# naver/multi-hmr

Measured on AMD Instinct MI355X. Metric: images/sec (whole node) ViT-L 896x896 bs32, higher is better.
Workload: dtype f16; 1 GPU; multiHMR_896_L full forward: dinov2_vitl14 896x896, 32 images/GPU, 8 pinned persons/image -> HPH (depth 2) -> SMPL-X LBS; image-sharded x1; global_batch=32, parallelism=dp1 (images)

## Files before the change

multi_hmr_amd/csrc/attention.hip:

```cpp
#include <stdlib.h>
#include <type_traits>
#include "mhmr_common.h"
#include "mhmr_internal.h"

namespace {

__device__ __forceinline__ float max_lane32(float v) {
    const auto r = __builtin_amdgcn_permlane32_swap(__float_as_uint(v), __float_as_uint(v), false, false);
    return fmaxf(__uint_as_float(r[0]), __uint_as_float(r[1]));
}

constexpr int KB = 64;
#ifndef MHMR_ATTN_DEFAULT_VARIANT
#define MHMR_ATTN_DEFAULT_VARIANT 6
#endif
constexpr int KV_TILE_BYTES = KB * 64 * 2;
constexpr float BAND = 8.f;

template <int DT, int NW, int RING, int MODE>
__device__ __forceinline__ void attn_body(
    const void* __restrict__ qk_, const void* __restrict__ vt_, void* __restrict__ out_, int T, int Tp, int C, int H, int nqt,
    float limit, int* __restrict__ flags, int ldo, int o8, const int bid) {
    typedef typename Op<DT>::T Tt;
    typedef typename Op<DT>::V8 V8;
    typedef typename Op<DT>::V4 V4;
    extern __shared__ __attribute__((aligned(16))) char smem[];

    const int tid = threadIdx.x, lane = tid & 63;
    const int w = __builtin_amdgcn_readfirstlane(tid >> 6);
    const int hi = lane >> 5, l31 = lane & 31;

    const int qt = bid % nqt, bh = bid / nqt;
    const int b = bh / H, h = bh - b * H;
    constexpr int QB = 32 * NW;
    if (qt * QB >= T) {
        if constexpr (MODE == 3) {
            if (lane == 0) flags[4 * bid + w] = 0;
        }
        return;
    }

    const Tt* qk = (const Tt*)qk_;
    const Tt* vt = (const Tt*)vt_;
    const int ldq = 2 * C;
    const size_t row0 = (size_t)b * Tp;

    const int q_row = qt * QB + 32 * w + l31;
    const bool active = qt * QB + 32 * w < T;
    const bool in_buf = qt * QB + 32 * w < Tp;
    V8 qf[4] = {};
    if (in_buf) {
        const Tt* qp = qk + (row0 + q_row) * ldq + h * 64 + 8 * hi;
#pragma unroll
        for (int ks = 0; ks < 4; ++ks) qf[ks] = *(const V8*)(qp + 16 * ks);
        if (q_row >= T) {
#pragma unroll
            for (int ks = 0; ks < 4; ++ks) qf[ks] = V8{};
        }
    }

    constexpr int PASSES = 8 / NW, ROWS_PER_PASS = 8 * NW;
    constexpr int OPS = 2 * PASSES;
    const int srow = tid >> 3;
    const int schunk = (tid & 7) ^ ((tid >> 4) & 7);
    const Tt* k_src = qk + (row0 + srow) * ldq + C + h * 64 + schunk * 8;
    const Tt* v_src = vt + ((size_t)(b * H + h) * 64 + srow) * Tp + schunk * 8;
    auto stage = [&](int j, int buf) {
        char* sk = smem + buf * (2 * KV_TILE_BYTES) + w * 1024;
        char* sv = sk + KV_TILE_BYTES;
        const Tt* kp = k_src + (size_t)j * KB * ldq;
        const Tt* vp = v_src + j * KB;
#pragma unroll
        for (int ps = 0; ps < PASSES; ++ps) glds16(kp + (size_t)(ROWS_PER_PASS * ps) * ldq, sk + ps * (ROWS_PER_PASS * 128));
#pragma unroll
        for (int ps = 0; ps < PASSES; ++ps) glds16(vp + (size_t)(ROWS_PER_PASS * ps) * Tp, sv + ps * (ROWS_PER_PASS * 128));
    };

    const int fsw = (lane >> 1) & 7;

    f32x16 o[2];
#pragma unroll
    for (int i = 0; i < 2; ++i)
#pragma unroll
        for (int r = 0; r < 16; ++r) o[i][r] = 0.f;
    float m_ref = MODE == 1 ? -1e30f : 0.f, r_run = -INFINITY, l_run = 0.f;
    bool bad = false;

    const bool tail1 = MODE == 3 && (T & (KB - 1)) == 1 && T > KB;
    const int ntile = tail1 ? T / KB : (T + KB - 1) / KB;
#pragma unroll
    for (int t = 0; t < RING - 1; ++t) stage(t < ntile ? t : ntile - 1, t);
    int buf = 0, nbuf = RING - 1;
    for (int j = 0; j < ntile; ++j) {
        if constexpr (RING == 2) asm volatile("s_waitcnt vmcnt(0) lgkmcnt(0)" ::: "memory");
        else if constexpr (OPS * (RING - 2) == 2) asm volatile("s_waitcnt vmcnt(2) lgkmcnt(0)" ::: "memory");
        else if constexpr (OPS * (RING - 2) == 4) asm volatile("s_waitcnt vmcnt(4) lgkmcnt(0)" ::: "memory");
        else if constexpr (OPS * (RING - 2) == 6) asm volatile("s_waitcnt vmcnt(6) lgkmcnt(0)" ::: "memory");
        else asm volatile("s_waitcnt vmcnt(8) lgkmcnt(0)" ::: "memory");
        static_assert(OPS * (RING - 2) <= 8, "extend the counted waits");
        __builtin_amdgcn_s_barrier();
        __builtin_amdgcn_sched_barrier(0);
        const char* sk = smem + buf * (2 * KV_TILE_BYTES);
        const char* sv = sk + KV_TILE_BYTES;
        const int nbuf_now = nbuf;
        buf = buf == RING - 1 ? 0 : buf + 1;
        nbuf = nbuf == RING - 1 ? 0 : nbuf + 1;
        if (!active) {
            stage(j + RING - 1 < ntile ? j + RING - 1 : ntile - 1, nbuf_now);
            continue;
        }
        f32x16 s[2];
        {
            const float init = MODE == 1 ? 0.f : -m_ref;
#pragma unroll
            for (int sub = 0; sub < 2; ++sub)
#pragma unroll
                for (int r = 0; r < 16; ++r) s[sub][r] = init;
        }
        __builtin_amdgcn_s_setprio(1);
#pragma unroll
        for (int ks = 0; ks < 4; ++ks) {
            V8 kf[2];
#pragma unroll
            for (int sub = 0; sub < 2; ++sub) kf[sub] = *(const V8*)(sk + (32 * sub + l31) * 128 + (((2 * ks + hi) ^ fsw) * 16));
#pragma unroll
            for (int sub = 0; sub < 2; ++sub) s[sub] = Op<DT>::mfma32(kf[sub], qf[ks], s[sub]);
        }
        __builtin_amdgcn_s_setprio(0);
        stage(j + RING - 1 < ntile ? j + RING - 1 : ntile - 1, nbuf_now);
        __builtin_amdgcn_sched_barrier(0);
        if (j * KB + KB > T) {
#pragma unroll
            for (int sub = 0; sub < 2; ++sub)
#pragma unroll
                for (int r = 0; r < 16; ++r)
                    if (j * KB + 32 * sub + crow(r, hi) >= T) s[sub][r] = -INFINITY;
        }
        if (MODE != 3 || j == 0) {
            float mt = s[0][0];
#pragma unroll
            for (int r = 1; r < 16; ++r) mt = fmaxf(mt, s[0][r]);
#pragma unroll
            for (int r = 0; r < 16; ++r) mt = fmaxf(mt, s[1][r]);
            mt = max_lane32(mt);
            if constexpr (MODE == 1) {
                const float m_new = fmaxf(m_ref, mt);
                if (!__all(m_new == m_ref)) {
                    const float alpha = __builtin_amdgcn_exp2f(m_ref - m_new);
                    l_run *= alpha;
#pragma unroll
                    for (int i = 0; i < 2; ++i)
#pragma unroll
                        for (int r = 0; r < 16; ++r) o[i][r] *= alpha;
                    m_ref = m_new;
                }
#pragma unroll
                for (int sub = 0; sub < 2; ++sub)
#pragma unroll
                    for (int r = 0; r < 16; ++r) s[sub][r] -= m_ref;
            } else if constexpr (MODE == 2) {
                const float r_new = fmaxf(r_run, mt);
                if (!__all(r_new <= BAND && r_new >= -BAND)) {
                    const float delta = r_new;
                    const float alpha = r_run == -INFINITY ? 1.f : __builtin_amdgcn_exp2f(-delta);
                    l_run *= alpha;
#pragma unroll
                    for (int i = 0; i < 2; ++i)
#pragma unroll
                        for (int r = 0; r < 16; ++r) o[i][r] *= alpha;
#pragma unroll
                    for (int sub = 0; sub < 2; ++sub)
#pragma unroll
                        for (int r = 0; r < 16; ++r) s[sub][r] -= delta;
                    m_ref += delta;
                    r_run = 0.f;
                } else {
                    r_run = r_new;
                }
            } else {
#pragma unroll
                for (int sub = 0; sub < 2; ++sub)
#pragma unroll
                    for (int r = 0; r < 16; ++r) s[sub][r] -= mt;
                m_ref = mt;
            }
        }
        float psum0 = 0.f, psum1 = 0.f;
#pragma unroll
        for (int r = 0; r < 16; ++r) {
            s[0][r] = __builtin_amdgcn_exp2f(s[0][r]);
            s[1][r] = __builtin_amdgcn_exp2f(s[1][r]);
        }

        __builtin_amdgcn_s_setprio(1);
#pragma unroll
        for (int st = 0; st < 4; ++st) {
            V8 pf;
#pragma unroll
            for (int e = 0; e < 8; ++e) pf[e] = (Tt)s[st >> 1][8 * (st & 1) + e];
            {
                const u32x4 pw = __builtin_bit_cast(u32x4, pf);
                psum0 = Op<DT>::pair_sum(pw[0], psum0);
                psum1 = Op<DT>::pair_sum(pw[1], psum1);
                psum0 = Op<DT>::pair_sum(pw[2], psum0);
                psum1 = Op<DT>::pair_sum(pw[3], psum1);
            }
#pragma unroll
            for (int ds = 0; ds < 2; ++ds) {
                const V8 vf = *(const V8*)(sv + (32 * ds + l31) * 128 + (((2 * st + hi) ^ fsw) * 16));
                o[ds] = Op<DT>::mfma32(vf, pf, o[ds]);
            }
        }
        {
            const float psum = psum0 + psum1;
            l_run += psum;
            if constexpr (MODE == 3) bad |= !(psum <= limit);
        }
        __builtin_amdgcn_s_setprio(0);
    }

    if constexpr (MODE == 3) {
        if (tail1 && active) {
            int kl = T - 1, lane2 = lane;
            asm volatile("" : "+s"(kl), "+v"(lane2));
            const int hi2 = lane2 >> 5;
            const Tt* kp = qk + (row0 + kl) * ldq + C + h * 64 + 8 * hi2;
            float dot = 0.f;
#pragma unroll
            for (int ks = 0; ks < 4; ++ks) {
                const V8 kf = *(const V8*)(kp + 16 * ks);
#pragma unroll
                for (int e = 0; e < 8; ++e) dot = __builtin_fmaf((float)qf[ks][e], (float)kf[e], dot);
            }
            dot += __shfl_xor(dot, 32);
            const float p = __builtin_amdgcn_exp2f(dot - m_ref);
            bad |= !(p <= limit);
            if (hi == 0) l_run += p;
            const int klp = (kl & ~12) | ((kl & 4) << 1) | ((kl & 8) >> 1);
            float* vl = (float*)(smem + RING * 2 * KV_TILE_BYTES) + w * 64;
            vl[lane2] = (float)vt[((size_t)(b * H + h) * 64 + lane2) * Tp + klp];
            asm volatile("s_waitcnt lgkmcnt(0)" ::: "memory");
#pragma unroll
            for (int ds = 0; ds < 2; ++ds)
#pragma unroll
                for (int rg = 0; rg < 4; ++rg) {
                    const f32x4 v4 = *(const f32x4*)(vl + 32 * ds + 8 * rg + 4 * hi2);
#pragma unroll
                    for (int e = 0; e < 4; ++e) o[ds][4 * rg + e] = __builtin_fmaf(v4[e], p, o[ds][4 * rg + e]);
                }
        }
    }
    asm volatile("s_waitcnt vmcnt(0)" ::: "memory");
    if constexpr (MODE == 3) {
        static_assert(MODE != 3 || NW == 4, "four flags per workgroup");
        const bool anybad = __any(bad);
        if (lane == 0) flags[4 * bid + w] = anybad ? 1 : 0;
    }
    const float l_tot = l_run + __shfl_xor(l_run, 32);
    const float inv = active ? 1.0f / l_tot : 0.f;
    if (!in_buf) return;
    int lane3 = lane;
    asm volatile("" : "+v"(lane3));
    Tt* op = (Tt*)out_ + (row0 + (qt * QB + 32 * w + (lane3 & 31))) * (size_t)ldo + h * 64 + 4 * (lane3 >> 5);
    char* op8 = (char*)((Tt*)out_ + (row0 + (qt * QB + 32 * w + (lane3 & 31))) * (size_t)ldo) + o8 + h * 64 + 4 * (lane3 >> 5);
#pragma unroll
    for (int ds = 0; ds < 2; ++ds)
#pragma unroll
        for (int rg = 0; rg < 4; ++rg) {
            V4 v;
            float f[4];
#pragma unroll
            for (int e = 0; e < 4; ++e) { f[e] = o[ds][4 * rg + e] * inv; v[e] = (Tt)f[e]; }
            *(V4*)(op + 32 * ds + 8 * rg) = v;
            if (o8 > 0) *(uint32_t*)(op8 + 32 * ds + 8 * rg) = pack_bf8x4(f[0], f[1], f[2], f[3]);
        }
}

template <int DT, int NW, int RING, int MODE>
__global__ __launch_bounds__(64 * NW, NW == 4 ? 4 : 2) void attn_kernel(
    const void* __restrict__ qk_, const void* __restrict__ vt_, void* __restrict__ out_, int T, int Tp, int C, int H, int nqt,
    float limit, int* __restrict__ flags, int ldo, int o8) {
    attn_body<DT, NW, RING, MODE>(qk_, vt_, out_, T, Tp, C, H, nqt, limit, flags, ldo, o8, xcd_remap(blockIdx.x, gridDim.x));
}

constexpr int FALLBACK_SLICE = 16;
template <int DT>
__global__ __launch_bounds__(256, 4) void attn_fallback_kernel(const void* __restrict__ qk_, const void* __restrict__ vt_, void* __restrict__ out_,
                                                               int T, int Tp, int C, int H, int nqt, float limit, int* __restrict__ flags,
                                                               int ldo, int o8, int nwg) {
    __shared__ unsigned int smask;
    const int tid = threadIdx.x, wg = blockIdx.x * FALLBACK_SLICE + tid;
    if (tid < 64) {
        int any = 0;
        if (tid < FALLBACK_SLICE && wg < nwg) {
            const int4 f = *(const int4*)(flags + 4 * wg);
            any = (f.x | f.y | f.z | f.w) != 0;
        }
        const unsigned long long m = __ballot(any);
        if (tid == 0) smask = (unsigned int)m;
    }
    __syncthreads();
    unsigned int mm = smask;
    while (mm) {
        const int bit = __builtin_ctz(mm);
        mm &= mm - 1;
        attn_body<DT, 4, 2, 1>(qk_, vt_, out_, T, Tp, C, H, nqt, limit, nullptr, ldo, o8, blockIdx.x * FALLBACK_SLICE + bit);
        __syncthreads();
    }
}


template <int DT>
struct QBlock {
    typename Op<DT>::V8 qf[4];
    f32x16 o[2];
    float mneg;
    float l_run;
    bool bad;
};

template <int DT, int RING>
__global__ __launch_bounds__(256, 2) void attn64_kernel(const void* __restrict__ qk_, const void* __restrict__ vt_, void* __restrict__ out_,
                                                        int T, int Tp, int C, int H, int nqt, float limit, int* __restrict__ flags) {
    typedef typename Op<DT>::T Tt;
    typedef typename Op<DT>::V8 V8;
    typedef typename Op<DT>::V4 V4;
    extern __shared__ __attribute__((aligned(16))) char smem[];

    const int tid = threadIdx.x, lane = tid & 63;
    const int w = __builtin_amdgcn_readfirstlane(tid >> 6);
    const int hi = lane >> 5, l31 = lane & 31;
    const int bid = xcd_remap(blockIdx.x, gridDim.x);
    const int qt = bid % nqt, bh = bid / nqt;
    const int b = bh / H, h = bh - b * H;

    const Tt* qk = (const Tt*)qk_;
    const Tt* vt = (const Tt*)vt_;
    const int ldq = 2 * C;
    const size_t row0 = (size_t)b * Tp;
    const int qr0 = qt * 256 + 64 * w;
    const bool active = qr0 < T;
    QBlock<DT> A, Bq;
    auto init_block = [&](QBlock<DT>& x, int first_row) {
#pragma unroll
        for (int ks = 0; ks < 4; ++ks) x.qf[ks] = V8{};
        if (first_row < Tp) {
            const Tt* qp = qk + (row0 + first_row + l31) * ldq + h * 64 + 8 * hi;
#pragma unroll
            for (int ks = 0; ks < 4; ++ks) x.qf[ks] = *(const V8*)(qp + 16 * ks);
        }
#pragma unroll
        for (int i = 0; i < 2; ++i)
#pragma unroll
            for (int r = 0; r < 16; ++r) x.o[i][r] = 0.f;
        x.mneg = 0.f;
        x.l_run = 0.f;
        x.bad = false;
    };
    init_block(A, qr0);
    init_block(Bq, qr0 + 32);

    const int srow = tid >> 3;
    const int schunk = (tid & 7) ^ ((tid >> 4) & 7);
    const Tt* k_src = qk + (row0 + srow) * ldq + C + h * 64 + schunk * 8;
    const Tt* v_src = vt + ((size_t)(b * H + h) * 64 + srow) * Tp + schunk * 8;
    auto stage = [&](int j, int buf) {
        char* sk = smem + buf * (2 * KV_TILE_BYTES) + w * 1024;
        char* sv = sk + KV_TILE_BYTES;
        const Tt* kp = k_src + (size_t)j * KB * ldq;
        const Tt* vp = v_src + j * KB;
        glds16(kp, sk);
        glds16(kp + (size_t)32 * ldq, sk + 4096);
        glds16(vp, sv);
        glds16(vp + (size_t)32 * Tp, sv + 4096);
    };
    const int fsw = (lane >> 1) & 7;
    const bool tail1 = (T & (KB - 1)) == 1 && T > KB;
    const int ntile = tail1 ? T / KB : (T + KB - 1) / KB;
    const int nfull = tail1 ? ntile : T / KB;

    auto splat = [&](float m) {
        asm volatile("" : "+v"(m));
        f32x16 t;
#pragma unroll
        for (int r = 0; r < 16; ++r) t[r] = m;
        return t;
    };
    auto mask_block = [&](f32x16 (&s)[2], int j) {
#pragma unroll
        for (int sub = 0; sub < 2; ++sub)
#pragma unroll
            for (int r = 0; r < 16; ++r)
                if (j * KB + 32 * sub + crow(r, hi) >= T) s[sub][r] = -INFINITY;
    };
    auto level_block = [&](QBlock<DT>& x, f32x16 (&s)[2]) {
        float mt = s[0][0];
#pragma unroll
        for (int r = 1; r < 16; ++r) mt = fmaxf(mt, s[0][r]);
#pragma unroll
        for (int r = 0; r < 16; ++r) mt = fmaxf(mt, s[1][r]);
        mt = max_lane32(mt);
#pragma unroll
        for (int sub = 0; sub < 2; ++sub)
#pragma unroll
            for (int r = 0; r < 16; ++r) s[sub][r] -= mt;
        x.mneg = -mt;
    };
#pragma unroll
    for (int t = 0; t < RING - 1; ++t) stage(t < ntile ? t : ntile - 1, t);
    int buf = 0, nbuf = RING - 1;
    auto tile_begin = [&](const char*& sk, const char*& sv, int& nbuf_now) {
        if constexpr (RING == 2) asm volatile("s_waitcnt vmcnt(0) lgkmcnt(0)" ::: "memory");
        else if constexpr (RING == 3) asm volatile("s_waitcnt vmcnt(4) lgkmcnt(0)" ::: "memory");
        else asm volatile("s_waitcnt vmcnt(8) lgkmcnt(0)" ::: "memory");
        static_assert(RING >= 2 && RING <= 4, "counted waits");
        __builtin_amdgcn_s_barrier();
        __builtin_amdgcn_sched_barrier(0);
        sk = smem + buf * (2 * KV_TILE_BYTES);
        sv = sk + KV_TILE_BYTES;
        nbuf_now = nbuf;
        buf = buf == RING - 1 ? 0 : buf + 1;
        nbuf = nbuf == RING - 1 ? 0 : nbuf + 1;
    };
    auto tile = [&](int j, auto first_c, auto masked_c) {
        constexpr bool FIRST = decltype(first_c)::value, MASKED = decltype(masked_c)::value;
        const char *sk, *sv;
        int nbuf_now;
        tile_begin(sk, sv, nbuf_now);
        const int jn = j + RING - 1 < ntile ? j + RING - 1 : ntile - 1;
        if (!active) {
            stage(jn, nbuf_now);
            return;
        }
        V8 fr[2][2];
        auto rdK = [&](int bi, int ks) {
#pragma unroll
            for (int sub = 0; sub < 2; ++sub) fr[bi][sub] = *(const V8*)(sk + (32 * sub + l31) * 128 + (((2 * ks + hi) ^ fsw) * 16));
        };
        auto rdV = [&](int bi, int st) {
#pragma unroll
            for (int ds = 0; ds < 2; ++ds) fr[bi][ds] = *(const V8*)(sv + (32 * ds + l31) * 128 + (((2 * st + hi) ^ fsw) * 16));
        };
        f32x16 sA[2], sB[2];
        V8 pA[4], pB[4];
        float ps0 = 0.f, ps1 = 0.f;
        auto sm_quarter = [&](f32x16 (&s)[2], V8 (&pf)[4], int c) {
#pragma unroll
            for (int e = 0; e < 8; e += 2) {
                const float p0 = __builtin_amdgcn_exp2f(s[c >> 1][8 * (c & 1) + e]);
                const float p1 = __builtin_amdgcn_exp2f(s[c >> 1][8 * (c & 1) + e + 1]);
                ps0 += p0;
                ps1 += p1;
                pf[c][e] = (Tt)p0;
                pf[c][e + 1] = (Tt)p1;
            }
        };
        auto sm_close = [&](QBlock<DT>& x) {
            const float psum = ps0 + ps1;
            x.l_run += psum;
            x.bad |= !(psum <= limit);
            ps0 = 0.f;
            ps1 = 0.f;
        };
        rdK(0, 0);
        const f32x16 initA = splat(A.mneg);
#define MHMR_STEP_SPLIT() __builtin_amdgcn_sched_barrier(0)
#pragma unroll
        for (int ks = 0; ks < 4; ++ks) {
            rdK((ks + 1) & 1, ks < 3 ? ks + 1 : 0);
#pragma unroll
            for (int sub = 0; sub < 2; ++sub) sA[sub] = Op<DT>::mfma32(fr[ks & 1][sub], A.qf[ks], ks == 0 ? initA : sA[sub]);
            if (ks == 0) stage(jn, nbuf_now);
            MHMR_STEP_SPLIT();
        }
        if constexpr (MASKED) mask_block(sA, j);
        if constexpr (FIRST) level_block(A, sA);
        if constexpr (MASKED || FIRST) __builtin_amdgcn_sched_barrier(0);
        const f32x16 initB = splat(Bq.mneg);
#pragma unroll
        for (int ks = 0; ks < 4; ++ks) {
#pragma unroll
            for (int sub = 0; sub < 2; ++sub) sB[sub] = Op<DT>::mfma32(fr[ks & 1][sub], Bq.qf[ks], ks == 0 ? initB : sB[sub]);
            MHMR_STEP_SPLIT();
            if (ks < 3) rdK((ks + 1) & 1, ks + 1);
            else rdV(0, 0);
            sm_quarter(sA, pA, ks);
            MHMR_STEP_SPLIT();
        }
        sm_close(A);
        if constexpr (MASKED) mask_block(sB, j);
        if constexpr (FIRST) level_block(Bq, sB);
        if constexpr (MASKED || FIRST) __builtin_amdgcn_sched_barrier(0);
#pragma unroll
        for (int st = 0; st < 4; ++st) {
#pragma unroll
            for (int ds = 0; ds < 2; ++ds) A.o[ds] = Op<DT>::mfma32(fr[st & 1][ds], pA[st], A.o[ds]);
            MHMR_STEP_SPLIT();
            rdV((st + 1) & 1, st < 3 ? st + 1 : 0);
            sm_quarter(sB, pB, st);
            MHMR_STEP_SPLIT();
        }
        sm_close(Bq);
#pragma unroll
        for (int st = 0; st < 4; ++st) {
            if (st < 3) rdV((st + 1) & 1, st + 1);
#pragma unroll
            for (int ds = 0; ds < 2; ++ds) Bq.o[ds] = Op<DT>::mfma32(fr[st & 1][ds], pB[st], Bq.o[ds]);
            MHMR_STEP_SPLIT();
        }
#undef MHMR_STEP_SPLIT
    };
    {
        using TT = std::true_type;
        using FF = std::false_type;
        if (nfull > 0) tile(0, TT{}, FF{});
        else tile(0, TT{}, TT{});
        for (int j = 1; j < nfull; ++j) tile(j, FF{}, FF{});
        if (ntile > nfull && nfull > 0) tile(nfull, FF{}, TT{});
    }

    float* vl = (float*)(smem + RING * 2 * KV_TILE_BYTES) + w * 64;
    auto tail_block = [&](QBlock<DT>& x, int kl) {
        int lane2 = lane;
        asm volatile("" : "+s"(kl), "+v"(lane2));
        const int hi2 = lane2 >> 5;
        const Tt* kp = qk + (row0 + kl) * ldq + C + h * 64 + 8 * hi2;
        float dot = 0.f;
#pragma unroll
        for (int ks = 0; ks < 4; ++ks) {
            const V8 kf = *(const V8*)(kp + 16 * ks);
#pragma unroll
            for (int e = 0; e < 8; ++e) dot = __builtin_fmaf((float)x.qf[ks][e], (float)kf[e], dot);
        }
        dot += __shfl_xor(dot, 32);
        const float p = __builtin_amdgcn_exp2f(dot + x.mneg);
        x.bad |= !(p <= limit);
        if (hi == 0) x.l_run += p;
#pragma unroll
        for (int ds = 0; ds < 2; ++ds)
#pragma unroll
            for (int rg = 0; rg < 4; ++rg) {
                const f32x4 v4 = *(const f32x4*)(vl + 32 * ds + 8 * rg + 4 * hi2);
#pragma unroll
                for (int e = 0; e < 4; ++e) x.o[ds][4 * rg + e] = __builtin_fmaf(v4[e], p, x.o[ds][4 * rg + e]);
            }
    };
    if (tail1 && active) {
        const int kl = T - 1;
        const int klp = (kl & ~12) | ((kl & 4) << 1) | ((kl & 8) >> 1);
        vl[lane] = (float)vt[((size_t)(b * H + h) * 64 + lane) * Tp + klp];
        asm volatile("s_waitcnt lgkmcnt(0)" ::: "memory");
        tail_block(A, kl);
        tail_block(Bq, kl);
    }
    asm volatile("s_waitcnt vmcnt(0)" ::: "memory");
    const int nqt1 = (Tp + 127) / 128, qt1 = 2 * qt + (w >> 1);
    auto finish_block = [&](QBlock<DT>& x, int blk) {
        const int first_row = qr0 + 32 * blk;
        const bool anybad = __any(x.bad);
        if (lane == 0 && qt1 < nqt1) flags[4 * (bh * nqt1 + qt1) + 2 * (w & 1) + blk] = (anybad && first_row < T) ? 1 : 0;
        const float l_tot = x.l_run + __shfl_xor(x.l_run, 32);
        const float inv = first_row < T ? 1.0f / l_tot : 0.f;
        if (first_row >= Tp) return;
        int lane3 = lane;
        asm volatile("" : "+v"(lane3));
        Tt* op = (Tt*)out_ + (row0 + (first_row + (lane3 & 31))) * C + h * 64 + 4 * (lane3 >> 5);
#pragma unroll
        for (int ds = 0; ds < 2; ++ds)
#pragma unroll
            for (int rg = 0; rg < 4; ++rg) {
                V4 v;
#pragma unroll
                for (int e = 0; e < 4; ++e) v[e] = (Tt)(x.o[ds][4 * rg + e] * inv);
                *(V4*)(op + 32 * ds + 8 * rg) = v;
            }
    };
    finish_block(A, 0);
    finish_block(Bq, 1);
}

template <int DT>
__device__ __forceinline__ float cls_dot2(uint32_t a, uint32_t b, float acc) {
    typedef typename Op<DT>::V2 V2;
    if constexpr (DT == MHMR_DT_F16) return __builtin_amdgcn_fdot2(__builtin_bit_cast(V2, a), __builtin_bit_cast(V2, b), acc, false);
    else return __builtin_amdgcn_fdot2_f32_bf16(__builtin_bit_cast(V2, a), __builtin_bit_cast(V2, b), acc, false);
}
template <int DT>
__device__ __forceinline__ float cls_half(uint32_t w, int hi) {
    typedef typename Op<DT>::T Tt;
    return (float)__builtin_bit_cast(Tt, (uint16_t)(hi ? w >> 16 : w));
}
__device__ __forceinline__ void cls_gload64(u32x4& d0, u32x4& d1, u32x4& d2, u32x4& d3, const void* p) {
    asm volatile("global_load_dwordx4 %0, %4, off\n\tglobal_load_dwordx4 %1, %4, off offset:16\n\t"
                 "global_load_dwordx4 %2, %4, off offset:32\n\tglobal_load_dwordx4 %3, %4, off offset:48"
                 : "=&v"(d0), "=&v"(d1), "=&v"(d2), "=&v"(d3) : "v"(p) : "memory");
}
template <int N>
__device__ __forceinline__ void cls_wait(u32x4* a, u32x4* b) {
    asm volatile("s_waitcnt vmcnt(%8)" : "+v"(a[0]), "+v"(a[1]), "+v"(a[2]), "+v"(a[3]), "+v"(b[0]), "+v"(b[1]), "+v"(b[2]), "+v"(b[3]) : "n"(N) : "memory");
}
template <int DT>
__device__ __forceinline__ void attn_cls_role(const void* __restrict__ qk_, const void* __restrict__ vt_, void* __restrict__ out_, int T, int Tp,
                                              int C, int H, int nqt, int* __restrict__ flags, int ldo, int bh, int w, int lane, char* smem) {
    typedef typename Op<DT>::T Tt;
    const int b = bh / H, h = bh - b * H;
    const Tt* qk = (const Tt*)qk_;
    const Tt* vt = (const Tt*)vt_;
    const int ldq = 2 * C;
    const size_t row0 = (size_t)b * Tp;
    const int key = lane & 31, half = lane >> 5;
    const Tt* kbase = qk + (row0 + key) * ldq + C + h * 64 + 32 * half;
    const Tt* vbase = vt + ((size_t)(b * H + h) * 64 + lane) * Tp;
    const int nst = (T + 31) / 32, last = nst - 1;
    const int nmine = (nst - w + 3) / 4;
    u32x4 q4[4], ka[4], va[4], kb[4], vb[4];
    auto issue = [&](int st, u32x4* k4, u32x4* v4) {
        if (st > last) st = last;
        cls_gload64(k4[0], k4[1], k4[2], k4[3], kbase + (size_t)st * 32 * ldq);
        cls_gload64(v4[0], v4[1], v4[2], v4[3], vbase + st * 32);
    };
    float m_ref = 0.f, l_lane = 0.f, o = 0.f;
    bool first = true;
    auto step = [&](int st, const u32x4* k4, const u32x4* v4) {
        float sa = 0.f, sb = 0.f;
#pragma unroll
        for (int i = 0; i < 4; ++i) {
            sa = cls_dot2<DT>(k4[i][0], q4[i][0], sa);
            sb = cls_dot2<DT>(k4[i][1], q4[i][1], sb);
            sa = cls_dot2<DT>(k4[i][2], q4[i][2], sa);
            sb = cls_dot2<DT>(k4[i][3], q4[i][3], sb);
        }
        float sc = sa + sb;
        sc += __shfl_xor(sc, 32);
        if (st * 32 + key >= T) sc = -INFINITY;
        if (first || __any(sc > m_ref + 64.f)) {
            float mx = sc;
#pragma unroll
            for (int d = 16; d >= 1; d >>= 1) mx = fmaxf(mx, __shfl_xor(mx, d));
            const float f = first ? 0.f : __builtin_amdgcn_exp2f(m_ref - mx);
            o *= f;
            l_lane *= f;
            m_ref = mx;
            first = false;
        }
        const float pv = __builtin_amdgcn_exp2f(sc - m_ref);
        l_lane += pv;
        const int pbits = __builtin_bit_cast(int, pv);
#pragma unroll
        for (int c = 0; c < 32; ++c) {
            const int src = (c & ~12) | ((c & 4) << 1) | ((c & 8) >> 1);
            const float pc = __builtin_bit_cast(float, __builtin_amdgcn_readlane(pbits, src));
            o = __builtin_fmaf(pc, cls_half<DT>(v4[c >> 3][(c >> 1) & 3], c & 1), o);
        }
    };
    cls_gload64(q4[0], q4[1], q4[2], q4[3], qk + (row0 + T - 1) * ldq + h * 64 + 32 * half);
    issue(w, ka, va);
    for (int i = 0; i < nmine; i += 2) {
        const int st = w + 4 * i;
        issue(st + 4, kb, vb);
        cls_wait<8>(ka, va);
        asm volatile("" : "+v"(q4[0]), "+v"(q4[1]), "+v"(q4[2]), "+v"(q4[3]));
        step(st, ka, va);
        if (i + 1 < nmine) {
            issue(st + 8, ka, va);
            cls_wait<8>(kb, vb);
            step(st + 4, kb, vb);
        }
    }
    cls_wait<0>(ka, va);
    cls_wait<0>(kb, vb);
    float l = half == 0 ? l_lane : 0.f;
#pragma unroll
    for (int d = 32; d >= 1; d >>= 1) l += __shfl_xor(l, d);
    float* part = (float*)smem;
    part[w * 66 + lane] = o;
    if (lane == 0) { part[w * 66 + 64] = m_ref; part[w * 66 + 65] = l; }
    __syncthreads();
    if (w != 0) return;
    float M = part[64];
#pragma unroll
    for (int i = 1; i < 4; ++i) M = fmaxf(M, part[i * 66 + 64]);
    float O = 0.f, L = 0.f;
#pragma unroll
    for (int i = 0; i < 4; ++i) {
        const float f = __builtin_amdgcn_exp2f(part[i * 66 + 64] - M);
        O = __builtin_fmaf(part[i * 66 + lane], f, O);
        L = __builtin_fmaf(part[i * 66 + 65], f, L);
    }
    ((Tt*)out_)[(row0 + T - 1) * (size_t)ldo + h * 64 + lane] = (Tt)(O / L);
    if (flags != nullptr)
        for (int i = 4 * (T / 128) + lane; i < 4 * nqt; i += 64) flags[4 * bh * nqt + i] = 0;
}

template <int DT, bool EARLY, int RING, int NQB>
__device__ __forceinline__ void attn16_tail(const typename Op<DT>::T* __restrict__ qk, const typename Op<DT>::T* __restrict__ vt, void* __restrict__ out_,
                                            int T, int Tp, int C, int H, float limit, int* __restrict__ flags, int ldo, int o8, int bid, int qt, int b, int h,
                                            int w, int lane, int j15, int g, int tid, char* smem, size_t row0, int ldq, bool active, bool in_buf) {
    typedef typename Op<DT>::T Tt;
    typedef typename Op<DT>::V8 V8;
    typedef typename Op<DT>::V4 V4;
    constexpr int QB = 128;
    V8 qf[2][2] = {};
#pragma unroll
    for (int qb = 0; qb < NQB; ++qb) {
        const int q_row = qt * QB + 32 * w + 16 * qb + j15;
        if (in_buf) {
            const Tt* qp = qk + (row0 + q_row) * ldq + h * 64 + 8 * g;
#pragma unroll
            for (int ks = 0; ks < 2; ++ks) qf[qb][ks] = *(const V8*)(qp + 32 * ks);
            if (q_row >= T) { qf[qb][0] = V8{}; qf[qb][1] = V8{}; }
        }
    }
    const int srow = tid >> 3;
    const int kchunk = (tid & 7) ^ (((srow >> 1) & 3) | (((srow >> 4) & 1) << 2));
    const int vchunk = (tid & 7) ^ ((srow >> 1) & 7);
    const uint32_t k_lane = (uint32_t)(srow * ldq + kchunk * 8) * 2u;
    const uint32_t v_lane = (uint32_t)(srow * Tp + vchunk * 8) * 2u;
    const char* k_base = (const char*)(qk + row0 * ldq + C + h * 64);
    const char* v_base = (const char*)(vt + (size_t)(b * H + h) * 64 * Tp);
    auto stage = [&](int jt, int buf) {
        char* sk = smem + buf * (2 * KV_TILE_BYTES) + w * 1024;
        char* sv = sk + KV_TILE_BYTES;
        const char* kp = k_base + (size_t)jt * KB * ldq * 2;
        const char* vp = v_base + (size_t)jt * KB * 2;
        uint32_t kl = k_lane, vl_ = v_lane;
        asm volatile("" : "+v"(kl), "+v"(vl_));
        const char* kp1 = kp + (size_t)32 * ldq * 2;
        const char* vp1 = vp + (size_t)32 * Tp * 2;
        asm volatile("" : "+s"(kp1), "+s"(vp1));
        glds16(kp + kl, sk);
        glds16(kp1 + kl, sk + 4096);
        glds16(vp + vl_, sv);
        glds16(vp1 + vl_, sv + 4096);
    };
    const int krow = j15 + (j15 & 8);
    const int kb_g = (g & 1) * 4 + (g >> 1) * 16;
    const int kf_sw = g ^ (((krow >> 1) & 3) | (((krow >> 4) & 1) << 2));
    const int vf_sw = g ^ ((j15 >> 1) & 7);
    int kofs[2] = {krow * 128 + kf_sw * 16, krow * 128 + (kf_sw ^ 4) * 16};
    int vofs[2] = {j15 * 128 + vf_sw * 16, j15 * 128 + (vf_sw ^ 4) * 16};

    f32x4 o[4][2];
#pragma unroll
    for (int db = 0; db < 4; ++db)
#pragma unroll
        for (int qb = 0; qb < NQB; ++qb) o[db][qb] = (f32x4){0.f, 0.f, 0.f, 0.f};
    float m_ref[2] = {0.f, 0.f}, l_run[2] = {0.f, 0.f};
    bool bad = false;
    const bool tail1 = (T & (KB - 1)) == 1 && T > KB;
    const int ntile = tail1 ? T / KB : (T + KB - 1) / KB;
    char* lone = smem + RING * 2 * KV_TILE_BYTES + 4 * 256;
    if (tail1 && w == 0) {
        const int kl = T - 1;
        const int klp = (kl & ~12) | ((kl & 4) << 1) | ((kl & 8) >> 1);
        __builtin_amdgcn_global_load_lds((const __attribute__((address_space(1))) void*)(vt + ((size_t)(b * H + h) * 64 + lane) * Tp + (klp & ~1)),
                                         (__attribute__((address_space(3))) void*)(lone + 128), 4, 0, 0);
        if (lane < 32)
            __builtin_amdgcn_global_load_lds((const __attribute__((address_space(1))) void*)(qk + (row0 + kl) * ldq + C + h * 64 + 2 * lane),
                                             (__attribute__((address_space(3))) void*)lone, 4, 0, 0);
    }
    stage(0, 0);
    if constexpr (RING == 3) stage(ntile > 1 ? 1 : 0, 1);
    int buf = 0, nbuf = RING - 1;
    for (int jt = 0; jt < ntile; ++jt) {
        if constexpr (RING == 3) asm volatile("s_waitcnt vmcnt(4) lgkmcnt(0)" ::: "memory");
        else asm volatile("s_waitcnt vmcnt(0) lgkmcnt(0)" ::: "memory");
        __builtin_amdgcn_s_barrier();
        __builtin_amdgcn_sched_barrier(0);
        const char* sk = smem + buf * (2 * KV_TILE_BYTES);
        const char* sv = sk + KV_TILE_BYTES;
        const int nbuf_now = nbuf;
        if constexpr (RING == 3) { buf = buf == 2 ? 0 : buf + 1; nbuf = nbuf == 2 ? 0 : nbuf + 1; }
        else { buf ^= 1; nbuf ^= 1; }
        const int jnext = jt + RING - 1 < ntile ? jt + RING - 1 : ntile - 1;
        if (!active) {
            stage(jnext, nbuf_now);
            continue;
        }
        if constexpr (EARLY) {
            stage(jnext, nbuf_now);
            __builtin_amdgcn_sched_barrier(0);
        }
        f32x4 sc[2][2][2];
#pragma unroll
        for (int m = 0; m < 2; ++m)
#pragma unroll
            for (int xy = 0; xy < 2; ++xy)
#pragma unroll
                for (int qb = 0; qb < NQB; ++qb) sc[m][xy][qb] = (f32x4){-m_ref[qb], -m_ref[qb], -m_ref[qb], -m_ref[qb]};
        __builtin_amdgcn_s_setprio(1);
#pragma unroll
        for (int ks = 0; ks < 2; ++ks)
#pragma unroll
            for (int m = 0; m < 2; ++m) {
                V8 kf[2];
#pragma unroll
                for (int xy = 0; xy < 2; ++xy) kf[xy] = *(const V8*)(sk + kofs[ks] + (32 * m + 8 * xy) * 128);
#pragma unroll
                for (int xy = 0; xy < 2; ++xy)
#pragma unroll
                    for (int qb = 0; qb < NQB; ++qb) sc[m][xy][qb] = Op<DT>::mfma16(kf[xy], qf[qb][ks], sc[m][xy][qb]);
            }
        __builtin_amdgcn_s_setprio(0);
        if constexpr (!EARLY) stage(jnext, nbuf_now);
        __builtin_amdgcn_sched_barrier(0);
        if (jt * KB + KB > T) {
#pragma unroll
            for (int m = 0; m < 2; ++m)
#pragma unroll
                for (int xy = 0; xy < 2; ++xy)
#pragma unroll
                    for (int r = 0; r < 4; ++r)
                        if (jt * KB + 32 * m + 8 * xy + kb_g + r >= T) { sc[m][xy][0][r] = -INFINITY; sc[m][xy][1][r] = -INFINITY; }
        }
        if (jt == 0) {
#pragma unroll
            for (int qb = 0; qb < NQB; ++qb) {
                float mt = sc[0][0][qb][0];
#pragma unroll
                for (int m = 0; m < 2; ++m)
#pragma unroll
                    for (int xy = 0; xy < 2; ++xy)
#pragma unroll
                        for (int r = 0; r < 4; ++r) mt = fmaxf(mt, sc[m][xy][qb][r]);
                mt = fmaxf(mt, __shfl_xor(mt, 16));
                mt = fmaxf(mt, __shfl_xor(mt, 32));
#pragma unroll
                for (int m = 0; m < 2; ++m)
#pragma unroll
                    for (int xy = 0; xy < 2; ++xy)
#pragma unroll
                        for (int r = 0; r < 4; ++r) sc[m][xy][qb][r] -= mt;
                m_ref[qb] = mt;
            }
        }
#pragma unroll
        for (int m = 0; m < 2; ++m)
#pragma unroll
            for (int xy = 0; xy < 2; ++xy)
#pragma unroll
                for (int qb = 0; qb < NQB; ++qb)
#pragma unroll
                    for (int r = 0; r < 4; ++r) sc[m][xy][qb][r] = __builtin_amdgcn_exp2f(sc[m][xy][qb][r]);
        float psum[2] = {0.f, 0.f};
        __builtin_amdgcn_s_setprio(1);
#pragma unroll
        for (int m = 0; m < 2; ++m) {
            V8 pf[2];
#pragma unroll
            for (int qb = 0; qb < NQB; ++qb) {
#pragma unroll
                for (int e = 0; e < 4; ++e) { pf[qb][e] = (Tt)sc[m][0][qb][e]; pf[qb][4 + e] = (Tt)sc[m][1][qb][e]; }
                const u32x4 pw = __builtin_bit_cast(u32x4, pf[qb]);
                psum[qb] = Op<DT>::pair_sum(pw[0], psum[qb]);
                psum[qb] = Op<DT>::pair_sum(pw[1], psum[qb]);
                psum[qb] = Op<DT>::pair_sum(pw[2], psum[qb]);
                psum[qb] = Op<DT>::pair_sum(pw[3], psum[qb]);
            }
#pragma unroll
            for (int db = 0; db < 4; ++db) {
                const V8 vf = *(const V8*)(sv + vofs[m] + db * 2048);
#pragma unroll
                for (int qb = 0; qb < NQB; ++qb) o[db][qb] = Op<DT>::mfma16(vf, pf[qb], o[db][qb]);
            }
        }
#pragma unroll
        for (int qb = 0; qb < NQB; ++qb) {
            l_run[qb] += psum[qb];
            bad |= !(psum[qb] <= limit);
        }
        __builtin_amdgcn_s_setprio(0);
    }

    if (tail1 && active) {
        int kl = T - 1, lane2 = lane;
        asm volatile("" : "+s"(kl), "+v"(lane2));
        const int g2 = lane2 >> 4;
        const Tt* kp = (const Tt*)lone + 8 * g2;
        float dot[2] = {0.f, 0.f};
#pragma unroll
        for (int ks = 0; ks < 2; ++ks) {
            const V8 kf = *(const V8*)(kp + 32 * ks);
#pragma unroll
            for (int qb = 0; qb < NQB; ++qb)
#pragma unroll
                for (int e = 0; e < 8; ++e) dot[qb] = __builtin_fmaf((float)qf[qb][ks][e], (float)kf[e], dot[qb]);
        }
        const int klp = (kl & ~12) | ((kl & 4) << 1) | ((kl & 8) >> 1);
        float* vl = (float*)(smem + RING * 2 * KV_TILE_BYTES) + w * 64;
        {
            const uint32_t raw = ((const uint32_t*)(lone + 128))[lane2];
            const uint16_t bits = (uint16_t)((klp & 1) ? raw >> 16 : raw);
            vl[lane2] = (float)__builtin_bit_cast(Tt, bits);
        }
        asm volatile("s_waitcnt lgkmcnt(0)" ::: "memory");
#pragma unroll
        for (int qb = 0; qb < NQB; ++qb) {
            float d = dot[qb];
            d += __shfl_xor(d, 16);
            d += __shfl_xor(d, 32);
            const float p = __builtin_amdgcn_exp2f(d - m_ref[qb]);
            bad |= !(p <= limit);
            if (g2 == 0) l_run[qb] += p;
#pragma unroll
            for (int db = 0; db < 4; ++db) {
                const f32x4 v4 = *(const f32x4*)(vl + 16 * db + 4 * g2);
#pragma unroll
                for (int e = 0; e < 4; ++e) o[db][qb][e] = __builtin_fmaf(v4[e], p, o[db][qb][e]);
            }
        }
    }
    asm volatile("s_waitcnt vmcnt(0)" ::: "memory");
    {
        const bool anybad = __any(bad);
        if (lane == 0) flags[4 * bid + w] = anybad ? 1 : 0;
    }
    if (!in_buf) return;
    int lane3 = lane;
    asm volatile("" : "+v"(lane3));
#pragma unroll
    for (int qb = 0; qb < NQB; ++qb) {
        float l_tot = l_run[qb];
        l_tot += __shfl_xor(l_tot, 16);
        l_tot += __shfl_xor(l_tot, 32);
        const float inv = active ? 1.0f / l_tot : 0.f;
        Tt* op = (Tt*)out_ + (row0 + (qt * QB + 32 * w + 16 * qb + (lane3 & 15))) * (size_t)ldo + h * 64 + 4 * (lane3 >> 4);
        char* op8 = (char*)((Tt*)out_ + (row0 + (qt * QB + 32 * w + 16 * qb + (lane3 & 15))) * (size_t)ldo) + o8 + h * 64 + 4 * (lane3 >> 4);
#pragma unroll
        for (int db = 0; db < 4; ++db) {
            V4 v;
            float f[4];
#pragma unroll
            for (int e = 0; e < 4; ++e) { f[e] = o[db][qb][e] * inv; v[e] = (Tt)f[e]; }
            *(V4*)(op + 16 * db) = v;
            if (o8 > 0) *(uint32_t*)(op8 + 16 * db) = pack_bf8x4(f[0], f[1], f[2], f[3]);
        }
    }
}

template <int DT, bool EARLY = false, int RING = 2, bool CLSQ = false>
__global__ __launch_bounds__(256, RING == 2 ? 4 : 3) void attn16_kernel(const void* __restrict__ qk_, const void* __restrict__ vt_, void* __restrict__ out_,
                                                        int T, int Tp, int C, int H, int nqt, float limit, int* __restrict__ flags, int ldo,
                                                        int o8, int ncls = 0, int nbh = 0) {
    typedef typename Op<DT>::T Tt;
    typedef typename Op<DT>::V8 V8;
    typedef typename Op<DT>::V4 V4;
    extern __shared__ __attribute__((aligned(16))) char smem[];
    constexpr int QB = 128;
    const int tid = threadIdx.x, lane = tid & 63;
    const int w = __builtin_amdgcn_readfirstlane(tid >> 6);
    const int j15 = lane & 15, g = lane >> 4;
    int bid;
    if constexpr (CLSQ) {
        if ((int)blockIdx.x < ncls) {
            if ((int)blockIdx.x >= nbh) return;
            int ln = lane;
            asm volatile("" : "+v"(ln));
            attn_cls_role<DT>(qk_, vt_, out_, T, Tp, C, H, nqt, flags, ldo, (int)blockIdx.x, w, ln, smem);
            return;
        }
        const int nfull = T / QB;
        const int r = xcd_remap((int)blockIdx.x - ncls, (int)gridDim.x - ncls);
        bid = (r / nfull) * nqt + r % nfull;
    } else {
        bid = xcd_remap(blockIdx.x, gridDim.x);
    }
    const int qt = bid % nqt, bh = bid / nqt;
    const int b = bh / H, h = bh - b * H;
    if (qt * QB >= T) {
        if (lane == 0) flags[4 * bid + w] = 0;
        return;
    }
    const Tt* qk = (const Tt*)qk_;
    const Tt* vt = (const Tt*)vt_;
    const int ldq = 2 * C;
    const size_t row0 = (size_t)b * Tp;
    const bool active = qt * QB + 32 * w < T;
    const bool in_buf = qt * QB + 32 * w < Tp;
    if (T - qt * QB <= 16) attn16_tail<DT, EARLY, RING, 1>(qk, vt, out_, T, Tp, C, H, limit, flags, ldo, o8, bid, qt, b, h, w, lane, j15, g, tid, smem, row0, ldq, active, in_buf);
    else attn16_tail<DT, EARLY, RING, 2>(qk, vt, out_, T, Tp, C, H, limit, flags, ldo, o8, bid, qt, b, h, w, lane, j15, g, tid, smem, row0, ldq, active, in_buf);
}

template <bool EARLY = false, int RING = 2>
int launch_attn16(const void* qk, const void* vt, void* out, int B, int T, int Tp, int C, int H, int dtype, float limit, int* flags,
                  hipStream_t s, int ldo, int o8) {
    const int nqt = (Tp + 127) / 128;
    const int grid = nqt * H * B;
    const size_t lds = RING * 2 * KV_TILE_BYTES + 4 * 256 + 384;
    if (dtype == MHMR_DT_F16)
        hipLaunchKernelGGL((attn16_kernel<MHMR_DT_F16, EARLY, RING>), dim3(grid), dim3(256), lds, s, qk, vt, out, T, Tp, C, H, nqt, limit, flags, ldo, o8);
    else
        hipLaunchKernelGGL((attn16_kernel<MHMR_DT_BF16, EARLY, RING>), dim3(grid), dim3(256), lds, s, qk, vt, out, T, Tp, C, H, nqt, limit, flags, ldo, o8);
    MHMR_CHECK_LAUNCH();
    return 0;
}

int launch_attn16_clsq(const void* qk, const void* vt, void* out, int B, int T, int Tp, int C, int H, int dtype, float limit, int* flags,
                       hipStream_t s, int ldo, int o8) {
    if (T % 128 != 1 || T < 129 || o8 != 0) return launch_attn16<false, 2>(qk, vt, out, B, T, Tp, C, H, dtype, limit, flags, s, ldo, o8);
    const int nqt = (Tp + 127) / 128, nbh = B * H;
    const int ncls = (nbh + 7) / 8 * 8;
    const int grid = ncls + (T / 128) * nbh;
    const size_t lds = 2 * 2 * KV_TILE_BYTES + 4 * 256 + 384;
    if (dtype == MHMR_DT_F16)
        hipLaunchKernelGGL((attn16_kernel<MHMR_DT_F16, false, 2, true>), dim3(grid), dim3(256), lds, s, qk, vt, out, T, Tp, C, H, nqt, limit, flags, ldo, o8, ncls, nbh);
    else
        hipLaunchKernelGGL((attn16_kernel<MHMR_DT_BF16, false, 2, true>), dim3(grid), dim3(256), lds, s, qk, vt, out, T, Tp, C, H, nqt, limit, flags, ldo, o8, ncls, nbh);
    MHMR_CHECK_LAUNCH();
    return 0;
}

template <int RING>
int launch_attn64(const void* qk, const void* vt, void* out, int B, int T, int Tp, int C, int H, int dtype, float limit, int* flags,
                  hipStream_t s) {
    const int nqt = (Tp + 255) / 256;
    const int grid = nqt * H * B;
    const size_t lds = RING * 2 * KV_TILE_BYTES + 4 * 256;
    if (dtype == MHMR_DT_F16)
        hipLaunchKernelGGL((attn64_kernel<MHMR_DT_F16, RING>), dim3(grid), dim3(256), lds, s, qk, vt, out, T, Tp, C, H, nqt, limit, flags);
    else
        hipLaunchKernelGGL((attn64_kernel<MHMR_DT_BF16, RING>), dim3(grid), dim3(256), lds, s, qk, vt, out, T, Tp, C, H, nqt, limit, flags);
    MHMR_CHECK_LAUNCH();
    return 0;
}

int launch_attn_fallback(const void* qk, const void* vt, void* out, int B, int T, int Tp, int C, int H, int dtype, float limit, int* flags,
                         hipStream_t s, int ldo = 0, int o8 = 0) {
    if (ldo <= 0) ldo = C;
    const int nqt = (Tp + 127) / 128, nwg = nqt * H * B;
    const int grid = (nwg + FALLBACK_SLICE - 1) / FALLBACK_SLICE;
    const size_t lds = 2 * 2 * KV_TILE_BYTES + 4 * 256;
    if (dtype == MHMR_DT_F16)
        hipLaunchKernelGGL((attn_fallback_kernel<MHMR_DT_F16>), dim3(grid), dim3(256), lds, s, qk, vt, out, T, Tp, C, H, nqt, limit, flags, ldo, o8, nwg);
    else
        hipLaunchKernelGGL((attn_fallback_kernel<MHMR_DT_BF16>), dim3(grid), dim3(256), lds, s, qk, vt, out, T, Tp, C, H, nqt, limit, flags, ldo, o8, nwg);
    MHMR_CHECK_LAUNCH();
    return 0;
}

template <int NW, int RING, int MODE>
int launch_attn(const void* qk, const void* vt, void* out, int B, int T, int Tp, int C, int H, int dtype, float limit, int* flags,
                hipStream_t s, int ldo = 0, int o8 = 0) {
    if (ldo <= 0) ldo = C;
    constexpr int QB = 32 * NW;
    const int nqt = (Tp + QB - 1) / QB;
    const int grid = nqt * H * B;
    const size_t lds = RING * 2 * KV_TILE_BYTES + NW * 256;
    if (dtype == MHMR_DT_F16)
        hipLaunchKernelGGL((attn_kernel<MHMR_DT_F16, NW, RING, MODE>), dim3(grid), dim3(64 * NW), lds, s, qk, vt, out, T, Tp, C, H, nqt, limit, flags, ldo, o8);
    else
        hipLaunchKernelGGL((attn_kernel<MHMR_DT_BF16, NW, RING, MODE>), dim3(grid), dim3(64 * NW), lds, s, qk, vt, out, T, Tp, C, H, nqt, limit, flags, ldo, o8);
    MHMR_CHECK_LAUNCH();
    return 0;
}

}

int mhmr_attention_flag_count_impl(int B, int Tp, int H) { return 4 * ((Tp + 127) / 128) * H * B; }

int mhmr_launch_attention_pitch(const void* qk, const void* vt, void* out, int B, int T, int Tp, int C, int H, int dtype, float limit_log2,
                                int variant, int* flags, hipStream_t s, int ldo, int o8);
int mhmr_launch_attention_ex(const void* qk, const void* vt, void* out, int B, int T, int Tp, int C, int H, int dtype, float limit_log2,
                             int variant, int* flags, hipStream_t s) {
    return mhmr_launch_attention_pitch(qk, vt, out, B, T, Tp, C, H, dtype, limit_log2, variant, flags, s, C, 0);
}
int mhmr_launch_attention_pitch(const void* qk, const void* vt, void* out, int B, int T, int Tp, int C, int H, int dtype, float limit_log2,
                                int variant, int* flags, hipStream_t s, int ldo, int o8) {
    if ((ldo != C || o8 != 0) && (variant < 6 || variant > 10 || ldo < C || o8 < 0 || (o8 > 0 && (o8 < 2 * C || o8 + C > 2 * ldo)))) return MHMR_ERR_BAD_ARG;
    if (C != H * 64 || Tp % 64 || T > Tp || T <= 0 || limit_log2 < 0.f || limit_log2 > 15.f) return MHMR_ERR_BAD_SHAPE;
    if ((variant == 0 || (variant >= 6 && variant <= 10)) && flags == nullptr) return MHMR_ERR_BAD_ARG;
    const float limit = exp2f(limit_log2);
    prof_begin(PROF_ATTN, s);
    int rc = 0;
    switch (variant) {
        case 0: {
            rc = launch_attn<4, 2, 3>(qk, vt, out, B, T, Tp, C, H, dtype, limit, flags, s);
            if (!rc) rc = launch_attn_fallback(qk, vt, out, B, T, Tp, C, H, dtype, limit, flags, s);
            break;
        }
        case 1: rc = launch_attn<4, 2, 1>(qk, vt, out, B, T, Tp, C, H, dtype, limit, nullptr, s); break;
        case 2: rc = launch_attn<4, 2, 2>(qk, vt, out, B, T, Tp, C, H, dtype, limit, nullptr, s); break;
        case 3: rc = launch_attn<8, 3, 2>(qk, vt, out, B, T, Tp, C, H, dtype, limit, nullptr, s); break;
        case 4:
        case 5: {
            if (flags == nullptr) return MHMR_ERR_BAD_ARG;
            rc = variant == 4 ? launch_attn64<3>(qk, vt, out, B, T, Tp, C, H, dtype, limit, flags, s)
                              : launch_attn64<2>(qk, vt, out, B, T, Tp, C, H, dtype, limit, flags, s);
            if (!rc) rc = launch_attn_fallback(qk, vt, out, B, T, Tp, C, H, dtype, limit, flags, s);
            break;
        }
        case 6:
        case 7:
        case 8:
        case 9: {
            if (flags == nullptr) return MHMR_ERR_BAD_ARG;
            rc = variant == 6 ? launch_attn16<false, 2>(qk, vt, out, B, T, Tp, C, H, dtype, limit, flags, s, ldo, o8)
               : variant == 7 ? launch_attn16<true, 2>(qk, vt, out, B, T, Tp, C, H, dtype, limit, flags, s, ldo, o8)
               : variant == 8 ? launch_attn16<false, 3>(qk, vt, out, B, T, Tp, C, H, dtype, limit, flags, s, ldo, o8)
                              : launch_attn16<true, 3>(qk, vt, out, B, T, Tp, C, H, dtype, limit, flags, s, ldo, o8);
            if (!rc) rc = launch_attn_fallback(qk, vt, out, B, T, Tp, C, H, dtype, limit, flags, s, ldo, o8);
            break;
        }
        case 10: {
            rc = launch_attn16_clsq(qk, vt, out, B, T, Tp, C, H, dtype, limit, flags, s, ldo, o8);
            if (!rc) rc = launch_attn_fallback(qk, vt, out, B, T, Tp, C, H, dtype, limit, flags, s, ldo, o8);
            break;
        }
        default: return MHMR_ERR_BAD_ARG;
    }
    prof_end(PROF_ATTN, s, 4.0 * B * H * (double)T * T * 64);
    return rc;
}

int mhmr_launch_attention(const void* qk, const void* vt, void* out, int B, int T, int Tp, int C, int H, int dtype, int* flags,
                          hipStream_t s, int ldo, int o8) {
    static const char* v = getenv("MHMR_ATTN_VARIANT");
    const int variant = v ? atoi(v) : (flags ? MHMR_ATTN_DEFAULT_VARIANT : 2);
    return mhmr_launch_attention_pitch(qk, vt, out, B, T, Tp, C, H, dtype, 15.f, variant, flags, s, ldo > 0 ? ldo : C, o8);
}
```

Measured before the change: 255.4 images/s.

## Split attention tile into two halves to overlap exp with PV MFMAs

Adds a HALF path to the attn16 kernel (now the default) that processes each full KV tile in two 32-key halves. Exponentials of the second half are interleaved with the PV MFMAs of the first half, and V loads are placed explicitly using sched_group_barrier. The aim is to hide transcendental and LDS latency behind matrix work inside a tile. The first tile and the tail tile still use the serial path, and the old behaviour stays reachable as variant 11. The cost is more live registers (vf, pf for both halves), which could hurt occupancy.

```diff
diff --git a/multi_hmr_amd/csrc/attention.hip b/multi_hmr_amd/csrc/attention.hip
--- a/multi_hmr_amd/csrc/attention.hip
+++ b/multi_hmr_amd/csrc/attention.hip
@@ -692,7 +692,7 @@
         for (int i = 4 * (T / 128) + lane; i < 4 * nqt; i += 64) flags[4 * bh * nqt + i] = 0;
 }
 
-template <int DT, bool EARLY, int RING, int NQB>
+template <int DT, bool EARLY, int RING, int NQB, bool HALF>
 __device__ __forceinline__ void attn16_tail(const typename Op<DT>::T* __restrict__ qk, const typename Op<DT>::T* __restrict__ vt, void* __restrict__ out_,
                                             int T, int Tp, int C, int H, float limit, int* __restrict__ flags, int ldo, int o8, int bid, int qt, int b, int h,
                                             int w, int lane, int j15, int g, int tid, char* smem, size_t row0, int ldq, bool active, bool in_buf) {
@@ -762,20 +762,25 @@
     stage(0, 0);
     if constexpr (RING == 3) stage(ntile > 1 ? 1 : 0, 1);
     int buf = 0, nbuf = RING - 1;
-    for (int jt = 0; jt < ntile; ++jt) {
+    auto enter = [&](int jt, int& nbuf_now, int& jnext) -> const char* {
         if constexpr (RING == 3) asm volatile("s_waitcnt vmcnt(4) lgkmcnt(0)" ::: "memory");
         else asm volatile("s_waitcnt vmcnt(0) lgkmcnt(0)" ::: "memory");
         __builtin_amdgcn_s_barrier();
         __builtin_amdgcn_sched_barrier(0);
         const char* sk = smem + buf * (2 * KV_TILE_BYTES);
-        const char* sv = sk + KV_TILE_BYTES;
-        const int nbuf_now = nbuf;
+        nbuf_now = nbuf;
         if constexpr (RING == 3) { buf = buf == 2 ? 0 : buf + 1; nbuf = nbuf == 2 ? 0 : nbuf + 1; }
         else { buf ^= 1; nbuf ^= 1; }
-        const int jnext = jt + RING - 1 < ntile ? jt + RING - 1 : ntile - 1;
+        jnext = jt + RING - 1 < ntile ? jt + RING - 1 : ntile - 1;
+        return sk;
+    };
+    auto tile_serial = [&](int jt) {
+        int nbuf_now, jnext;
+        const char* sk = enter(jt, nbuf_now, jnext);
+        const char* sv = sk + KV_TILE_BYTES;
         if (!active) {
             stage(jnext, nbuf_now);
-            continue;
+            return;
         }
         if constexpr (EARLY) {
             stage(jnext, nbuf_now);
@@ -870,6 +875,111 @@
             bad |= !(psum[qb] <= limit);
         }
         __builtin_amdgcn_s_setprio(0);
+    };
+    auto tile_half = [&](int jt) {
+        int nbuf_now, jnext;
+        const char* sk = enter(jt, nbuf_now, jnext);
+        const char* sv = sk + KV_TILE_BYTES;
+        if (!active) {
+            stage(jnext, nbuf_now);
+            return;
+        }
+        if constexpr (EARLY) {
+            stage(jnext, nbuf_now);
+            __builtin_amdgcn_sched_barrier(0);
+        }
+        f32x4 sc[2][2][2];
+#pragma unroll
+        for (int m = 0; m < 2; ++m)
+#pragma unroll
+            for (int xy = 0; xy < 2; ++xy)
+#pragma unroll
+                for (int qb = 0; qb < NQB; ++qb) sc[m][xy][qb] = (f32x4){-m_ref[qb], -m_ref[qb], -m_ref[qb], -m_ref[qb]};
+        auto scores = [&](int m) {
+#pragma unroll
+            for (int ks = 0; ks < 2; ++ks) {
+                V8 kf[2];
+#pragma unroll
+                for (int xy = 0; xy < 2; ++xy) kf[xy] = *(const V8*)(sk + kofs[ks] + (32 * m + 8 * xy) * 128);
+#pragma unroll
+                for (int xy = 0; xy < 2; ++xy)
+#pragma unroll
+                    for (int qb = 0; qb < NQB; ++qb) sc[m][xy][qb] = Op<DT>::mfma16(kf[xy], qf[qb][ks], sc[m][xy][qb]);
+            }
+        };
+        auto exps = [&](int m) {
+#pragma unroll
+            for (int xy = 0; xy < 2; ++xy)
+#pragma unroll
+                for (int qb = 0; qb < NQB; ++qb)
+#pragma unroll
+                    for (int r = 0; r < 4; ++r) sc[m][xy][qb][r] = __builtin_amdgcn_exp2f(sc[m][xy][qb][r]);
+        };
+        float psum[2] = {0.f, 0.f};
+        V8 pf[2][2], vf[2][4];
+        auto vload = [&](int m) {
+#pragma unroll
+            for (int db = 0; db < 4; ++db) vf[m][db] = *(const V8*)(sv + vofs[m] + db * 2048);
+        };
+        auto round_p = [&](int m) {
+#pragma unroll
+            for (int qb = 0; qb < NQB; ++qb) {
+#pragma unroll
+                for (int e = 0; e < 4; ++e) { pf[m][qb][e] = (Tt)sc[m][0][qb][e]; pf[m][qb][4 + e] = (Tt)sc[m][1][qb][e]; }
+                const u32x4 pw = __builtin_bit_cast(u32x4, pf[m][qb]);
+                psum[qb] = Op<DT>::pair_sum(pw[0], psum[qb]);
+                psum[qb] = Op<DT>::pair_sum(pw[1], psum[qb]);
+                psum[qb] = Op<DT>::pair_sum(pw[2], psum[qb]);
+                psum[qb] = Op<DT>::pair_sum(pw[3], psum[qb]);
+            }
+        };
+        auto pv = [&](int m) {
+#pragma unroll
+            for (int db = 0; db < 4; ++db)
+#pragma unroll
+                for (int qb = 0; qb < NQB; ++qb) o[db][qb] = Op<DT>::mfma16(vf[m][db], pf[m][qb], o[db][qb]);
+        };
+        constexpr int SG_MFMA = 0x8, SG_DSR = 0x100, SG_TRANS = 0x400;
+        __builtin_amdgcn_s_setprio(1);
+        scores(0);
+        scores(1);
+        __builtin_amdgcn_s_setprio(0);
+        if constexpr (!EARLY) stage(jnext, nbuf_now);
+        __builtin_amdgcn_sched_barrier(0);
+        exps(0);
+        __builtin_amdgcn_s_setprio(1);
+        vload(0);
+        round_p(0);
+        __builtin_amdgcn_sched_barrier(0);
+        pv(0);
+        exps(1);
+        vload(1);
+#pragma unroll
+        for (int i = 0; i < 4 * NQB; ++i) {
+            __builtin_amdgcn_sched_group_barrier(SG_MFMA, 1, 0);
+            __builtin_amdgcn_sched_group_barrier(SG_TRANS, 2, 0);
+            if (i == 2 * NQB - 1) __builtin_amdgcn_sched_group_barrier(SG_DSR, 4, 0);
+        }
+        __builtin_amdgcn_sched_barrier(0);
+        round_p(1);
+        pv(1);
+#pragma unroll
+        for (int qb = 0; qb < NQB; ++qb) {
+            l_run[qb] += psum[qb];
+            bad |= !(psum[qb] <= limit);
+        }
+        __builtin_amdgcn_s_setprio(0);
+    };
+    if constexpr (!HALF) {
+        for (int jt = 0; jt < ntile; ++jt) tile_serial(jt);
+    } else {
+        const int nfull = T / KB;
+        for (int jt = 0;;) {
+            tile_serial(jt);
+            if (jt > 0) break;
+            for (jt = 1; jt < nfull; ++jt) tile_half(jt);
+            if (jt >= ntile) break;
+        }
     }
 
     if (tail1 && active) {
@@ -938,7 +1048,7 @@
     }
 }
 
-template <int DT, bool EARLY = false, int RING = 2, bool CLSQ = false>
+template <int DT, bool EARLY = false, int RING = 2, bool CLSQ = false, bool HALF = true>
 __global__ __launch_bounds__(256, RING == 2 ? 4 : 3) void attn16_kernel(const void* __restrict__ qk_, const void* __restrict__ vt_, void* __restrict__ out_,
                                                         int T, int Tp, int C, int H, int nqt, float limit, int* __restrict__ flags, int ldo,
                                                         int o8, int ncls = 0, int nbh = 0) {
@@ -977,20 +1087,20 @@
     const size_t row0 = (size_t)b * Tp;
     const bool active = qt * QB + 32 * w < T;
     const bool in_buf = qt * QB + 32 * w < Tp;
-    if (T - qt * QB <= 16) attn16_tail<DT, EARLY, RING, 1>(qk, vt, out_, T, Tp, C, H, limit, flags, ldo, o8, bid, qt, b, h, w, lane, j15, g, tid, smem, row0, ldq, active, in_buf);
-    else attn16_tail<DT, EARLY, RING, 2>(qk, vt, out_, T, Tp, C, H, limit, flags, ldo, o8, bid, qt, b, h, w, lane, j15, g, tid, smem, row0, ldq, active, in_buf);
-}
-
-template <bool EARLY = false, int RING = 2>
+    if (T - qt * QB <= 16) attn16_tail<DT, EARLY, RING, 1, HALF>(qk, vt, out_, T, Tp, C, H, limit, flags, ldo, o8, bid, qt, b, h, w, lane, j15, g, tid, smem, row0, ldq, active, in_buf);
+    else attn16_tail<DT, EARLY, RING, 2, HALF>(qk, vt, out_, T, Tp, C, H, limit, flags, ldo, o8, bid, qt, b, h, w, lane, j15, g, tid, smem, row0, ldq, active, in_buf);
+}
+
+template <bool EARLY = false, int RING = 2, bool HALF = true>
 int launch_attn16(const void* qk, const void* vt, void* out, int B, int T, int Tp, int C, int H, int dtype, float limit, int* flags,
                   hipStream_t s, int ldo, int o8) {
     const int nqt = (Tp + 127) / 128;
     const int grid = nqt * H * B;
     const size_t lds = RING * 2 * KV_TILE_BYTES + 4 * 256 + 384;
     if (dtype == MHMR_DT_F16)
-        hipLaunchKernelGGL((attn16_kernel<MHMR_DT_F16, EARLY, RING>), dim3(grid), dim3(256), lds, s, qk, vt, out, T, Tp, C, H, nqt, limit, flags, ldo, o8);
+        hipLaunchKernelGGL((attn16_kernel<MHMR_DT_F16, EARLY, RING, false, HALF>), dim3(grid), dim3(256), lds, s, qk, vt, out, T, Tp, C, H, nqt, limit, flags, ldo, o8);
     else
-        hipLaunchKernelGGL((attn16_kernel<MHMR_DT_BF16, EARLY, RING>), dim3(grid), dim3(256), lds, s, qk, vt, out, T, Tp, C, H, nqt, limit, flags, ldo, o8);
+        hipLaunchKernelGGL((attn16_kernel<MHMR_DT_BF16, EARLY, RING, false, HALF>), dim3(grid), dim3(256), lds, s, qk, vt, out, T, Tp, C, H, nqt, limit, flags, ldo, o8);
     MHMR_CHECK_LAUNCH();
     return 0;
 }
@@ -1066,9 +1176,9 @@
 }
 int mhmr_launch_attention_pitch(const void* qk, const void* vt, void* out, int B, int T, int Tp, int C, int H, int dtype, float limit_log2,
                                 int variant, int* flags, hipStream_t s, int ldo, int o8) {
-    if ((ldo != C || o8 != 0) && (variant < 6 || variant > 10 || ldo < C || o8 < 0 || (o8 > 0 && (o8 < 2 * C || o8 + C > 2 * ldo)))) return MHMR_ERR_BAD_ARG;
+    if ((ldo != C || o8 != 0) && (variant < 6 || variant > 11 || ldo < C || o8 < 0 || (o8 > 0 && (o8 < 2 * C || o8 + C > 2 * ldo)))) return MHMR_ERR_BAD_ARG;
     if (C != H * 64 || Tp % 64 || T > Tp || T <= 0 || limit_log2 < 0.f || limit_log2 > 15.f) return MHMR_ERR_BAD_SHAPE;
-    if ((variant == 0 || (variant >= 6 && variant <= 10)) && flags == nullptr) return MHMR_ERR_BAD_ARG;
+    if ((variant == 0 || (variant >= 6 && variant <= 11)) && flags == nullptr) return MHMR_ERR_BAD_ARG;
     const float limit = exp2f(limit_log2);
     prof_begin(PROF_ATTN, s);
     int rc = 0;
@@ -1106,6 +1216,11 @@
             if (!rc) rc = launch_attn_fallback(qk, vt, out, B, T, Tp, C, H, dtype, limit, flags, s, ldo, o8);
             break;
         }
+        case 11: {
+            rc = launch_attn16<false, 2, false>(qk, vt, out, B, T, Tp, C, H, dtype, limit, flags, s, ldo, o8);
+            if (!rc) rc = launch_attn_fallback(qk, vt, out, B, T, Tp, C, H, dtype, limit, flags, s, ldo, o8);
+            break;
+        }
         default: return MHMR_ERR_BAD_ARG;
     }
     prof_end(PROF_ATTN, s, 4.0 * B * H * (double)T * T * 64);
```

Result: no change. 256.3 images/s, median of 6 (+0.3%).
